# rahulaggarwal965/vslam

Hardware: AMD Instinct MI355X
Metric: frame-pairs/sec (extract+match+RANSAC) @1280×720, 2k kp, 4096 hyp; 1/2/4/8 GPU (higher is better)
Workload: dtype u8/f32/f64; 1 GPU; C3: 1280x720, 2000 keypoints, 4096 hypotheses, batch 256 pairs per GPU, SURVEY 8(d) data: rotation + parallax, sub-pixel resampling, 40-45 % outlier matches; pairs_per_gpu=256, batches_in_flight=4

## Files before the change

vslam_amd/build.py:

```python
import os
import subprocess
import sys

HERE = os.path.dirname(os.path.abspath(__file__))
CSRC = os.path.join(HERE, "csrc")
LIB = os.path.join(HERE, "libvslam_amd.so")
SOURCES = ["capi.hip", "match.hip", "ransac_sets.hip", "ransac_solve.hip", "ransac_count.hip", "ransac_select.hip", "refit.hip", "refine.hip",
           "kdtree.hip", "gray.hip", "response.hip", "select.hip", "blur.hip",
           "brief.hip", "orb_grid.hip", "pose.hip", "assoc.hip", "map.hip", "world.hip", "render.hip", "multi.hip", "pipeline.hip"]
HEADERS = ["ctx.h", "introselect.h", "image_common.h", "ransac_svd.h", "ransac_residual.h", "refine_math.h", "world_select.h",
           os.path.join("..", "..", "include", "vslam_amd.h"),
           os.path.join("..", "..", "include", "vslam_brief_pattern_31.h")]
FLAGS = ["--offload-arch=gfx950", "-O3", "-std=c++17", "-ffp-contract=off", "-fPIC", "-Wall"]
EXTRA_FLAGS = {"response.hip": ["-fno-slp-vectorize"]}
OBJDIR = os.path.join(HERE, "_obj")


EXP_LIB = os.path.join(HERE, "libvslam_amd_exp.so")
EXP_OBJDIR = os.path.join(HERE, "_obj_exp")


def _compile(hipcc, src, verbose, objdir=None, extra=()):
    objdir = objdir or OBJDIR
    obj = os.path.join(objdir, src.replace(".hip", ".o"))
    deps = [os.path.join(CSRC, src)] + [os.path.join(CSRC, h) for h in HEADERS] + [os.path.abspath(__file__)]
    if os.path.exists(obj) and all(os.path.getmtime(d) <= os.path.getmtime(obj) for d in deps):
        return obj, None
    cmd = [hipcc] + FLAGS + list(extra) + EXTRA_FLAGS.get(src, []) + ["-c", "-o", obj, src]
    if verbose:
        print(" ".join(cmd))
    return obj, subprocess.Popen(cmd, cwd=CSRC)


def build(force=False, verbose=False, experiments=False):
    hipcc = os.environ.get("HIPCC", "/opt/rocm/bin/hipcc")
    objdir, lib, extra = (EXP_OBJDIR, EXP_LIB, ("-DVSLAM_EXPERIMENTS",)) if experiments else (OBJDIR, LIB, ())
    return _build(hipcc, objdir, lib, extra, force, verbose)


def _build(hipcc, OBJDIR, LIB, extra, force, verbose):
    os.makedirs(OBJDIR, exist_ok=True)
    if force:
        for f in os.listdir(OBJDIR):
            os.remove(os.path.join(OBJDIR, f))
    jobs = [_compile(hipcc, src, verbose, OBJDIR, extra) for src in SOURCES]
    failed = [obj for obj, proc in jobs if proc is not None and proc.wait() != 0]
    if failed:
        raise subprocess.CalledProcessError(1, "hipcc -c (" + ", ".join(os.path.basename(f) for f in failed) + ")")
    objs = [obj for obj, _ in jobs]
    if os.path.exists(LIB) and all(proc is None for _, proc in jobs) and all(
            os.path.getmtime(o) <= os.path.getmtime(LIB) for o in objs):
        return LIB
    cmd = [hipcc, "--offload-arch=gfx950", "-shared", "-fPIC", "-o", LIB] + objs
    if verbose:
        print(" ".join(cmd))
    subprocess.run(cmd, check=True)
    return LIB


HOST_LIB = os.path.join(HERE, "libvslam_host.so")
HOST_SRCS = [os.path.join(HERE, "host", f) for f in ("adapters.cpp", "kdtree_nodes.cpp", "ingest.cpp", "pointmap.cpp", "display.cpp")]
HOST_HDRS = [os.path.join(HERE, "host", "host_internal.h")]
INCLUDE = os.path.join(HERE, "..", "include")


def build_host(force=False, verbose=False):
    build(force=False)
    deps = HOST_SRCS + HOST_HDRS + [LIB] + [os.path.join(INCLUDE, "vslam", f) for f in os.listdir(os.path.join(INCLUDE, "vslam"))]
    if not force and os.path.exists(HOST_LIB) and all(os.path.getmtime(d) <= os.path.getmtime(HOST_LIB) for d in deps):
        return HOST_LIB
    cmd = ["g++", "-std=c++17", "-O2", "-fPIC", "-shared", "-Wall", "-pthread", "-o", HOST_LIB] + HOST_SRCS + [
        "-L" + HERE, "-lvslam_amd", "-Wl,-rpath,$ORIGIN"]
    if verbose:
        print(" ".join(cmd))
    subprocess.run(cmd, check=True)
    return HOST_LIB


if __name__ == "__main__":
    build(force="--force" in sys.argv, verbose=True)
    build_host(force="--force" in sys.argv, verbose=True)
    build(force="--force" in sys.argv, verbose=True, experiments=True)
    print(LIB)
    print(EXP_LIB)
    print(HOST_LIB)
```

vslam_amd/capi.py:

```python
import ctypes as C
import os

_HERE = os.path.dirname(os.path.abspath(__file__))
LIB_PATH = os.environ.get("VSLAM_AMD_LIB") or os.path.join(_HERE, "libvslam_amd.so")
EXP_LIB_PATH = os.path.join(_HERE, "libvslam_amd_exp.so")

OK = 0
ERRORS = {-1: "VSLAM_ERR_INVALID", -2: "VSLAM_ERR_HIP", -3: "VSLAM_ERR_NO_DEVICE",
          -4: "VSLAM_ERR_CAPACITY", -5: "VSLAM_ERR_DEGENERATE", -6: "VSLAM_ERR_COMM"}

SYMBOLS = [
    "vslam_ctx_create", "vslam_ctx_make_current", "vslam_ctx_destroy", "vslam_ctx_set_stream", "vslam_ctx_set_option", "vslam_ctx_synchronize", "vslam_ctx_wait",
    "vslam_last_error", "vslam_ctx_workspace_bytes", "vslam_version", "vslam_brief_pattern_31", "vslam_dev_alloc", "vslam_dev_free", "vslam_copy_h2d",
    "vslam_copy_d2h", "vslam_debug_stream_copy", "vslam_debug_valu_calib", "vslam_prof_enable", "vslam_prof_reset", "vslam_prof_count", "vslam_prof_get",
    "vslam_match_knn2_ratio", "vslam_ransac_sets", "vslam_ransac_fundamental", "vslam_ransac_solve",
    "vslam_ransac_evaluate", "vslam_refit_fundamental", "vslam_refine_pairs", "vslam_kdtree_build",
    "vslam_kdtree_radius", "vslam_kdtree_nearest", "vslam_kdtree_cell_table", "vslam_extract_features", "vslam_extract_features_grid", "vslam_triangulate_points", "vslam_frontend_pairs_pose", "vslam_pipeline_batches_redone", "vslam_corner_stats", "vslam_bgr2gray", "vslam_min_eigen",
    "vslam_good_features", "vslam_gaussian7", "vslam_orb_describe", "vslam_extract_Rt", "vslam_triangulate", "vslam_associate_map_points", "vslam_reprojection_filter",
    "vslam_match_features",
    "vslam_map_create", "vslam_map_destroy", "vslam_map_reset", "vslam_map_step", "vslam_map_view", "vslam_map_observations",
    "vslam_track_sequences",
    "vslam_world_create", "vslam_world_destroy", "vslam_world_reset", "vslam_world_step", "vslam_world_lift", "vslam_world_view",
    "vslam_map_attach_world", "vslam_world_render",
    "vslam_view_default", "vslam_view_look_at", "vslam_render_points", "vslam_map_render",
# ... 49 lines not shown
    def default(cls, width, height, lib=None):
        lib = lib or load_library()
        v = cls()
        rc = lib.vslam_view_default(C.c_int(width), C.c_int(height), C.byref(v))
        if rc != OK:
            raise VslamError(f"{ERRORS.get(rc, rc)}: vslam_view_default({width}, {height})")
        return v

    @classmethod
    def look_at(cls, eye, target, up, width, height, lib=None, **fields):
        lib = lib or load_library()
        v = cls.default(width, height, lib)
        d3 = C.c_double * 3
        rc = lib.vslam_view_look_at(d3(*[float(x) for x in eye]), d3(*[float(x) for x in target]), d3(*[float(x) for x in up]), v.mv)
        if rc != OK:
            raise VslamError(f"{ERRORS.get(rc, rc)}: vslam_view_look_at({eye}, {target}, {up})")
        for k, val in fields.items():
            if k in ("background_bgr", "frustum_bgr"):
                val = (C.c_uint8 * 3)(*val)
            setattr(v, k, val)
        return v

    def copy(self, **fields):
        v = type(self).from_buffer_copy(self)
        for k, val in fields.items():
            if k in ("background_bgr", "frustum_bgr"):
                val = (C.c_uint8 * 3)(*val)
            setattr(v, k, val)
        return v


def load_library(path=LIB_PATH):
    if not os.path.exists(path):
        raise VslamError(
            f"{path} is missing: run `python -m vslam_amd.build` (hipcc, gfx950). "
            "There is no CPU fallback.")
    lib = C.CDLL(path)
    lib.vslam_last_error.restype = C.c_char_p
    lib.vslam_version.restype = C.c_char_p
    return lib


def _ptr(t):
    if t is None:
        return C.c_void_p(0)
    if isinstance(t, int):
        return C.c_void_p(t)
    return C.c_void_p(t.data_ptr())


class Context:

    def __init__(self, device=0, use_torch_stream=True, lib=None):
        import torch
        self.torch = torch
        self.lib = lib if lib is not None else load_library()
        self.handle = C.c_void_p()
        rc = self.lib.vslam_ctx_create(C.c_int(device), C.byref(self.handle))
        if rc != OK:
            raise VslamError(f"vslam_ctx_create failed: {ERRORS.get(rc, rc)} (no HIP device? there is no CPU fallback)")
        self.device = torch.device("cuda", device)
        self.own_stream = not use_torch_stream
        if use_torch_stream:
            s = torch.cuda.current_stream(self.device)
            self._check(self.lib.vslam_ctx_set_stream(self.handle, C.c_void_p(s.cuda_stream)))

    def _ready(self):
        if getattr(self, "own_stream", True):
            self.torch.cuda.current_stream(self.device).synchronize()

    def close(self):
        if self.handle:
            self.lib.vslam_ctx_destroy(self.handle)
            self.handle = C.c_void_p()

    def __del__(self):
        try:
            self.close()
        except Exception:
            pass

    def _check(self, rc):
        if rc != OK:
            msg = self.lib.vslam_last_error(self.handle)
            raise VslamError(f"{ERRORS.get(rc, rc)}: {msg.decode() if msg else ''}")

    def _dev(self, t, dtype, name):
        torch = self.torch
        if t is None:
            return None
        if not (t.is_cuda and t.dtype == dtype and t.is_contiguous()):
            raise VslamError(f"{name}: need a contiguous cuda tensor of {dtype}, got {t.dtype} on {t.device}")
        return t

    def synchronize(self):
        self._check(self.lib.vslam_ctx_synchronize(self.handle))

    def corner_stats(self):
        a = (C.c_uint64 * 5)()
        self._check(self.lib.vslam_corner_stats(self.handle, a))
        return {"frames": int(a[0]), "px_per_frame": int(a[1]), "listed_pixels": int(a[2]), "frames_overflowed": int(a[3]),
                "pool_sets": int(a[4])}

    def workspace_bytes(self):
        n = C.c_size_t()
        self._check(self.lib.vslam_ctx_workspace_bytes(self.handle, C.byref(n)))
        return n.value

    OPT_RANSAC_ALL_SUMS = 1
    OPT_RANSAC_MIN_MATCHES = 2
    OPT_RANSAC_SOLVER = 3
    OPT_MATCH_SHAPE = 4
    OPT_CORNER_WINDOW_PCT = 5
    OPT_RANSAC_MIN_ITEMS = 6
    OPT_CORNER_LIST_CAP = 7
    OPT_MATCH_FORM = 8
    OPT_TREE_FORK = 9
    OPT_POSE_REFIT = 10
    OPT_POSE_REFINE = 11

    def set_option(self, option, value):
        self._check(self.lib.vslam_ctx_set_option(self.handle, C.c_int(option), C.c_int(int(value))))

    def prof_enable(self, on=True):
        self._check(self.lib.vslam_prof_enable(self.handle, C.c_int(1 if on else 0)))

    def prof_reset(self):
        self._check(self.lib.vslam_prof_reset(self.handle))

    def prof_report(self):
        n = self.lib.vslam_prof_count(self.handle)
        if n < 0:
            self._check(n)
        out = {}
        for i in range(n):
            name = C.create_string_buffer(128)
            ms = C.c_double()
            cnt = C.c_int64()
            self._check(self.lib.vslam_prof_get(self.handle, C.c_int(i), name, C.c_int(128), C.byref(ms), C.byref(cnt)))
            out[name.value.decode()] = (ms.value, cnt.value)
        return out

    def debug_detect(self, bgr, max_corners, width=None):
        torch = self.torch
        F, H = bgr.shape[0], bgr.shape[1]
        W = width if width is not None else bgr.shape[2]
        stride = bgr.shape[2] * (bgr.shape[3] if bgr.dim() == 4 else 1)
        xy = torch.zeros((F, max_corners, 2), dtype=torch.float32, device=bgr.device)
        n = torch.zeros((F,), dtype=torch.int32, device=bgr.device)
        self._ready()
        self._check(self.lib.vslam_debug_detect(self.handle, _ptr(bgr), C.c_int(F), C.c_int(W), C.c_int(H), C.c_int(stride),
                                                C.c_int(max_corners), C.c_int(max_corners), _ptr(xy), _ptr(n)))
        return xy, n

    def debug_valu_calib(self):
        self._check(self.lib.vslam_debug_valu_calib(self.handle))

    def debug_stream_copy(self, src, dst, bytes_per_lane):
        self._check(self.lib.vslam_debug_stream_copy(self.handle, _ptr(src), _ptr(dst), C.c_size_t(src.numel() * src.element_size()),
                                                     C.c_int(bytes_per_lane)))

    def match_knn2_ratio(self, desc1, n1, desc2, n2, want_knn=False):
        torch = self.torch
        B, K, _ = desc1.shape
        self._dev(desc1, torch.uint8, "desc1"); self._dev(desc2, torch.uint8, "desc2")
        self._dev(n1, torch.int32, "n1"); self._dev(n2, torch.int32, "n2")
        pairs = torch.empty((B, K, 2), dtype=torch.int32, device=desc1.device)
        m = torch.empty((B,), dtype=torch.int32, device=desc1.device)
        knn = torch.empty((B, K, 4), dtype=torch.int32, device=desc1.device) if want_knn else None
        self._check(self.lib.vslam_match_knn2_ratio(self.handle, _ptr(desc1), _ptr(n1), _ptr(desc2), _ptr(n2),
                                                    C.c_int(B), C.c_int(K), _ptr(pairs), _ptr(m), _ptr(knn)))
        return (pairs, m, knn) if want_knn else (pairs, m)

    def ransac_sets(self, seeds, m, hyp):
        torch = self.torch
        B = seeds.shape[0]
        self._dev(seeds, torch.int32, "seeds"); self._dev(m, torch.int32, "m")
        sets = torch.empty((B, hyp, 8), dtype=torch.int32, device=seeds.device)
        draws = torch.empty((B, hyp * 8), dtype=torch.int32, device=seeds.device)
        self._check(self.lib.vslam_ransac_sets(self.handle, _ptr(seeds), _ptr(m), C.c_int(B), C.c_int(hyp),
                                               _ptr(sets), _ptr(draws)))
        return sets

    def ransac_fundamental(self, xy1, xy2, pairs, m, sets, threshold):
        torch = self.torch
        B, K, _ = xy1.shape
        H = sets.shape[1]
        dev = xy1.device
        for t, dt, nm in ((xy1, torch.float32, "xy1"), (xy2, torch.float32, "xy2"), (pairs, torch.int32, "pairs"),
                          (m, torch.int32, "m"), (sets, torch.int32, "sets")):
            self._dev(t, dt, nm)
        out = dict(
            F=torch.zeros((B, 9), dtype=torch.float32, device=dev),
            mask=torch.zeros((B, K), dtype=torch.uint8, device=dev),
            best=torch.zeros((B, 4), dtype=torch.int32, device=dev),
            matches=torch.zeros((B, K, 2), dtype=torch.int32, device=dev),
            hypF=torch.zeros((B, H, 9), dtype=torch.float32, device=dev),
            hyp_count=torch.zeros((B, H), dtype=torch.int32, device=dev),
            hyp_sum=torch.zeros((B, H), dtype=torch.float32, device=dev),
        )
        self._check(self.lib.vslam_ransac_fundamental(
            self.handle, _ptr(xy1), _ptr(xy2), _ptr(pairs), _ptr(m), _ptr(sets), C.c_int(B), C.c_int(K),
            C.c_int(H), C.c_float(threshold), _ptr(out["F"]), _ptr(out["mask"]), _ptr(out["best"]),
            _ptr(out["matches"]), _ptr(out["hypF"]), _ptr(out["hyp_count"]), _ptr(out["hyp_sum"])))
        return out

    def ransac_evaluate(self, xy1, xy2, pairs, m, hypF, threshold):
        torch = self.torch
        B, K, _ = xy1.shape
        H = hypF.shape[1]
        dev = xy1.device
        for t, dt, nm in ((xy1, torch.float32, "xy1"), (xy2, torch.float32, "xy2"), (pairs, torch.int32, "pairs"),
                          (m, torch.int32, "m"), (hypF, torch.float32, "hypF")):
            self._dev(t, dt, nm)
        out = dict(
            F=torch.zeros((B, 9), dtype=torch.float32, device=dev),
            mask=torch.zeros((B, K), dtype=torch.uint8, device=dev),
            best=torch.zeros((B, 4), dtype=torch.int32, device=dev),
            matches=torch.zeros((B, K, 2), dtype=torch.int32, device=dev),
            hyp_count=torch.zeros((B, H), dtype=torch.int32, device=dev),
            hyp_sum=torch.zeros((B, H), dtype=torch.float32, device=dev),
        )
        self._check(self.lib.vslam_ransac_evaluate(
            self.handle, _ptr(xy1), _ptr(xy2), _ptr(pairs), _ptr(m), _ptr(hypF), C.c_int(B), C.c_int(K), C.c_int(H),
            C.c_float(threshold), _ptr(out["F"]), _ptr(out["mask"]), _ptr(out["best"]), _ptr(out["matches"]),
            _ptr(out["hyp_count"]), _ptr(out["hyp_sum"])))
        return out

    def refit_fundamental(self, xy1, xy2, matches, best, F, out=None, want_stats=True):
        torch = self.torch
        B, K, _ = xy1.shape
        for t, dt, nm in ((xy1, torch.float32, "xy1"), (xy2, torch.float32, "xy2"), (matches, torch.int32, "matches"),
                          (best, torch.int32, "best"), (F, torch.float32, "F"), (out, torch.float32, "out")):
            self._dev(t, dt, nm)
        if out is None:
            out = torch.empty((B, 9), dtype=torch.float32, device=xy1.device)
        stats = torch.empty((B, 4), dtype=torch.float64, device=xy1.device) if want_stats else None
        self._ready()
        self._check(self.lib.vslam_refit_fundamental(self.handle, _ptr(xy1), _ptr(xy2), _ptr(matches), _ptr(best), C.c_int(B),
                                                     C.c_int(K), _ptr(F), _ptr(out), _ptr(stats)))
        return out, stats

    def refine_pairs(self, xy1, xy2, matches, best, K, R, t, points4d, gate_sq=16.0, max_iterations=20, want_stats=True):
        import numpy as np
        torch = self.torch
        B, Kp, _ = xy1.shape
        for x, dt, nm in ((xy1, torch.float32, "xy1"), (xy2, torch.float32, "xy2"), (matches, torch.int32, "matches"),
                          (best, torch.int32, "best"), (R, torch.float32, "R"), (t, torch.float32, "t"),
                          (points4d, torch.float32, "points4d")):
            self._dev(x, dt, nm)
        Kh = np.ascontiguousarray(np.asarray(K, np.float32).reshape(9))
        c2 = torch.empty((B, 12), dtype=torch.float32, device=xy1.device)
        stats = torch.empty((B, 4), dtype=torch.float64, device=xy1.device) if want_stats else None
        self._ready()
        self._check(self.lib.vslam_refine_pairs(self.handle, _ptr(xy1), _ptr(xy2), _ptr(matches), _ptr(best), C.c_int(B), C.c_int(Kp),
                                                Kh.ctypes.data_as(C.c_void_p), C.c_float(gate_sq), C.c_int(max_iterations),
                                                _ptr(R), _ptr(t), _ptr(c2), _ptr(points4d), _ptr(stats)))
        return R, t, c2, points4d, stats

    def kdtree_build(self, xy, n):
        torch = self.torch
        B, K, _ = xy.shape
        self._dev(xy, torch.float32, "xy"); self._dev(n, torch.int32, "n")
        nodes = torch.full((B, K), -1, dtype=torch.int32, device=xy.device)
        self._check(self.lib.vslam_kdtree_build(self.handle, _ptr(xy), _ptr(n), C.c_int(B), C.c_int(K), _ptr(nodes)))
        return nodes

    def kdtree_radius(self, nodes, xy, n, queries, nq, radius, hit_cap=8):
        torch = self.torch
        B, K, _ = xy.shape
        Q = queries.shape[1]
        self._dev(nodes, torch.int32, "nodes"); self._dev(xy, torch.float32, "xy"); self._dev(n, torch.int32, "n")
        self._dev(queries, torch.float32, "queries"); self._dev(nq, torch.int32, "nq")
        hits = torch.full((B, Q, hit_cap), -1, dtype=torch.int32, device=xy.device)
        counts = torch.zeros((B, Q), dtype=torch.int32, device=xy.device)
        self._check(self.lib.vslam_kdtree_radius(self.handle, _ptr(nodes), _ptr(xy), _ptr(n), C.c_int(B), C.c_int(K),
                                                 _ptr(queries), _ptr(nq), C.c_int(Q), C.c_float(radius),
                                                 _ptr(hits), _ptr(counts), C.c_int(hit_cap)))
        return hits, counts

    def kdtree_nearest(self, nodes, xy, n, queries, nq, max_distance_sq=float("inf")):
        torch = self.torch
        B, K, _ = xy.shape
        Q = queries.shape[1]
        best = torch.full((B, Q), -2, dtype=torch.int32, device=xy.device)
        self._check(self.lib.vslam_kdtree_nearest(self.handle, _ptr(nodes), _ptr(xy), _ptr(n), C.c_int(B), C.c_int(K),
                                                  _ptr(queries), _ptr(nq), C.c_int(Q), C.c_float(max_distance_sq),
                                                  _ptr(best)))
        return best

    def bgr2gray(self, bgr):
        torch = self.torch
        F, H, W, _ = bgr.shape
        self._dev(bgr, torch.uint8, "bgr")
        gray = torch.empty((F, H, W), dtype=torch.uint8, device=bgr.device)
        self._check(self.lib.vslam_bgr2gray(self.handle, _ptr(bgr), C.c_int(F), C.c_int(W), C.c_int(H), C.c_int(3 * W), _ptr(gray)))
        return gray

    def min_eigen(self, gray):
        torch = self.torch
        F, H, W = gray.shape
        self._dev(gray, torch.uint8, "gray")
        eig = torch.empty((F, H, W), dtype=torch.float32, device=gray.device)
        self._check(self.lib.vslam_min_eigen(self.handle, _ptr(gray), C.c_int(F), C.c_int(W), C.c_int(H), _ptr(eig)))
        return eig

# ... 740 lines not shown
```

vslam_amd/csrc/ransac_count.hip:

```cpp
#include "ransac_residual.h"

namespace {
using namespace vs_ransac;

constexpr int kCntHyps = 128;
constexpr int kCntWaves = 8;
constexpr int kCntQueue = 320;
constexpr int kCntLdsMatches = 4096;
constexpr int kScreenMatches = 128;
constexpr int kScreenHyps = 128;
constexpr int kRankThreads = 512;
constexpr int kPilotHyps = kRankThreads / 64;
constexpr int kCandMax = 8;
constexpr float kCntTinyDD = 0x1p-120f;
constexpr int kFcmpOGT = 2, kFcmpOLT = 4, kFcmpULT = 12;
constexpr int kCntRec = 12;
typedef __attribute__((address_space(3))) volatile uint32_t cnt_queue_t;
static_assert(VSLAM_MAX_KP <= 65536, "queue words keep the match index in 16 bits");

__host__ __device__ constexpr int cnt_pad(int n) { return (n + 255) & ~255; }
constexpr int kHeadUncertified = -1;
__device__ __forceinline__ float cnt_sum_rel(int adds) { return fmaxf(0x1p-18f, (float)(13 + adds) * 0x1p-24f); }

struct CntBand {
// ... 662 lines not shown
            int knext = 0;
            if (lane == 0) knext = atomicAdd(&s_next, 1);
            int hh;
            {
                int kk = k, w = 0;
                while (w + 1 < kListWaves && kk >= s_nlist[w]) kk -= s_nlist[w++];
                hh = s_list[w * 64 + kk];
            }
            bound = max(bound, *(__attribute__((address_space(3))) const volatile int *)&s_bound);
            CntRec R;
            cnt_load_record(R, s_rec, hh);
            const int word = ZERO ? 0 : s_state[hh] >> 2;
            const int head_cnt = ZERO ? 0 : *(__attribute__((address_space(3))) const volatile int *)&s_cnt[hh];
            float head_sum = ZERO ? 0.f : s_part[hh];
            int cnt = 0, pot = word & 0xFFFF, seen = org;
            bool dropped = false, unk = false;
            v2f acc;
            acc.x = 0.f;
            acc.y = 0.f;
            for (int s = 0;; s++) {
                if (s >= nsub && (ZERO || s > nsub || !(word & kHeadMine))) break;
                const bool hd = !ZERO && s == nsub;
                const int pot_walk = pot;
                const int ix = (hd ? 0 : org + s * 256) + 4 * lane;
                const int il = min(ix, mpad - 4);
                const float4 X1 = *reinterpret_cast<const float4 *>(cx1 + il), Y1 = *reinterpret_cast<const float4 *>(cy1 + il);
                const float4 X2 = *reinterpret_cast<const float4 *>(cx2 + il), Y2 = *reinterpret_cast<const float4 *>(cy2 + il);
                if (hd || (s == nsub - 1 && part)) {
                    cnt_sub_block<true>(R, X1, Y1, X2, Y2, ix, hh, lane, hd ? n0 : m, cnt, q, qn, acc, s_unk, pot, unk);
                    seen += hd ? 0 : (m - org) & 255;
                } else {
                    cnt_sub_block<false>(R, X1, Y1, X2, Y2, ix, hh, lane, m, cnt, q, qn, acc, s_unk, pot, unk);
                    seen += 256;
                }
                while (qn >= 64) {
                    cnt_drain(q, qn - 64, 64, lane, s_rec, s_cnt, cx1, cy1, cx2, cy2, threshold);
                    qn -= 64;
                }
                if (hd) {
                    head_sum = 0.f;
                    pot = pot_walk;
                    break;
                }
                if (pot + (m - seen) < bound) {
                    dropped = true;
                    break;
                }
                if (seen < m && bound == floor_count && pot + (m - seen) == bound && !unk && R.beta >= 0.f && !(word & kHeadNoSum)) {
                    const float S = head_sum + __int_as_float(__builtin_amdgcn_readlane(__float_as_int(wave_sum_to_lane63(acc.x + acc.y)), 63));
                    const float ns = (float)seen;
                    const float err = (2.02f * R.beta * sqrtf(ns * S) + ns * R.beta * R.beta + sum_rel * S) * 1.0001f;
                    const float upper = ((S + err) + threshold * (float)(m - seen)) * 1.0001f;
                    if (upper < floor_sum * 0.9999f) {
                        dropped = true;
                        break;
                    }
                }
            }
            if (dropped) {
#ifdef VSLAM_EXPERIMENTS
                if (lane == 0) s_state[hh] = 2 | (seen << 2);
#else
                if (lane == 0) s_state[hh] = 2;
#endif
            } else {
                const float part_sum = head_sum + wave_sum_to_lane63(acc.x + acc.y);
                bool beaten = false;
                if (bound == floor_count && pot == bound && !unk && R.beta >= 0.f) {
                    const float S = __int_as_float(__builtin_amdgcn_readlane(__float_as_int(part_sum), 63));
                    const float ns = (float)m;
                    const float err = (2.02f * R.beta * sqrtf(ns * S) + ns * R.beta * R.beta + sum_rel * S) * 1.0001f;
                    beaten = (S + err) * 1.0001f < floor_sum * 0.9999f;
                }
                if (lane == 63) s_part[hh] = part_sum;
                const int certain = head_cnt + cnt;
                if (beaten) {
#ifdef VSLAM_EXPERIMENTS
                    if (lane == 0) s_state[hh] = 2 | (seen << 2);
#else
                    if (lane == 0) s_state[hh] = 2;
#endif
                } else if (lane == 0) {
                    if (cnt) atomicAdd(&s_cnt[hh], cnt);
                    if (certain > bound) {
                        atomicMax(&s_bound, certain);
                        atomicMax(&cbound[b], certain);
                    }
                }
                if (!beaten) bound = max(bound, certain);
            }
            k = __builtin_amdgcn_readfirstlane(knext);
        }
        if (qn > 0) cnt_drain(q, 0, qn, lane, s_rec, s_cnt, cx1, cy1, cx2, cy2, threshold);
    }
    __syncthreads();
    if (tid < nh) {
        const int st = s_state[tid] & 3;
        hyp_count[out] = st == 1 ? s_cnt[tid] : -1;
        int nan_bits = 0x7FC00000;
#ifdef VSLAM_EXPERIMENTS
        if (exit_payload && st != 1) nan_bits |= st == 2 ? min(s_state[tid] >> 2, 0x3FFFFF) : 0x3FFFFF;
#endif
        hyp_sum[out] = __int_as_float(nan_bits);
        const float S = st == 1 ? s_part[tid] : 0.f;
        float err = INFINITY;
        if (st == 1 && my_ok && !s_unk[tid]) {
            const double Sd = (double)S;
            const double rel = (double)cnt_sum_rel(2 * ((m - (ZERO ? 0 : n0) + 255) >> 8) + 9);
            err = (float)((2.02 * my_beta * sqrt((double)m * Sd) + (double)m * my_beta * my_beta + rel * Sd) * (1.0 + 0x1p-20));
        }
        reinterpret_cast<float2 *>(approx)[out] = make_float2(S, err);
    }
}

}

int vs_launch_ransac_count(vslam_ctx *ctx, const float *xy1, const float *xy2, const int32_t *pairs, const int32_t *m,
                           const float *hypF, int batch, int kp_stride, int hyp, float threshold, int32_t *hyp_count,
                           float *hyp_sum, float *approx) {
    const int min_m = ctx->ransac_min_matches;
    int rc;
    int32_t *cbound = nullptr, *pot0 = nullptr;
    float *rk = nullptr, *cmax = nullptr;
    const int kp_pad = cnt_pad(kp_stride);
    if ((rc = vs_arena_get(ctx, "ransac.cbound", sizeof(int32_t) * (size_t)batch, (void **)&cbound))) return rc;
    unsigned long long *sfloor = nullptr;
    if ((rc = vs_arena_get(ctx, "ransac.sfloor", sizeof(unsigned long long) * (size_t)batch, (void **)&sfloor))) return rc;
    static const bool no_sum_rule = VS_EXPERIMENT_ENV("VSLAM_RANSAC_NO_SUM_RULE") != nullptr;
    const bool from_zero = VS_EXPERIMENT_ENV("VSLAM_RANSAC_COUNT_FROM_ZERO") != nullptr;
#ifdef VSLAM_EXPERIMENTS
    const int exit_payload = VS_EXPERIMENT_ENV("VSLAM_RANSAC_COUNT_EXIT_PAYLOAD") != nullptr ? 1 : 0;
#endif
    int2 *head = nullptr;
    if ((rc = vs_arena_get(ctx, "ransac.head", sizeof(int2) * (size_t)batch * hyp, (void **)&head))) return rc;
    const unsigned long long *use_floor = no_sum_rule ? nullptr : sfloor;
    if ((rc = vs_arena_get(ctx, "ransac.pot0", sizeof(int32_t) * (size_t)batch * hyp, (void **)&pot0))) return rc;
    if ((rc = vs_arena_get(ctx, "ransac.rk", sizeof(float) * 4 * (size_t)kp_pad * batch, (void **)&rk))) return rc;
    if ((rc = vs_arena_get(ctx, "ransac.cmax", sizeof(float) * 2 * (size_t)batch, (void **)&cmax))) return rc;
    {
        VsProfScope ps(ctx, "ransac_rank_kernel");
        ransac_rank_kernel<<<batch, kRankThreads, 0, ctx->stream>>>(xy1, xy2, pairs, m, min_m, kp_stride, kp_pad, hyp, threshold, hypF,
                                                                    cbound, rk, cmax, sfloor);
    }
    {
        VsProfScope ps(ctx, "ransac_screen_kernel");
        dim3 grid(vs_div_up(hyp, kScreenHyps), batch);
        ransac_screen_kernel<<<grid, 256, 0, ctx->stream>>>(rk, kp_pad, m, min_m, kp_stride, hyp, threshold, hypF, cmax, cbound, pot0, head);
    }
    {
        VsProfScope ps(ctx, "ransac_cand_kernel");
        ransac_cand_kernel<<<batch, 64 * kCandMax, 0, ctx->stream>>>(rk, kp_pad, m, min_m, kp_stride, hyp, threshold, hypF, pot0,
                                                                     no_sum_rule ? 0 : 1, cbound, sfloor);
    }
    if (int arc = vs_aux_job_point(ctx, 4)) return arc;
    {
        VsProfScope ps(ctx, "ransac_count_kernel");
        const bool lds = kp_pad <= kCntLdsMatches;
        const size_t dyn = (lds ? sizeof(float) * 4 * (size_t)kp_pad : 0) + sizeof(uint32_t) * kCntQueue * kCntWaves;
        const size_t dyn_max = sizeof(float) * 4 * kCntLdsMatches + sizeof(uint32_t) * kCntQueue * kCntWaves;
        dim3 grid(vs_div_up(hyp, kCntHyps), batch);
#ifdef VSLAM_EXPERIMENTS
        if (from_zero) {
            if (dyn > 32 * 1024 && (rc = vs_allow_dynamic_lds(ctx, ransac_count_kernel<true, true>, "ransac_count_from_zero", dyn_max)))
                return rc;
            if (lds)
                ransac_count_kernel<true, true><<<grid, 64 * kCntWaves, dyn, ctx->stream>>>(
                    rk, kp_pad, m, min_m, kp_stride, hyp, threshold, hypF, pot0, head, cmax, hyp_count, hyp_sum, approx, cbound,
                    use_floor VS_CNT_PAYLOAD_ARG);
            else
                ransac_count_kernel<false, true><<<grid, 64 * kCntWaves, dyn, ctx->stream>>>(
                    rk, kp_pad, m, min_m, kp_stride, hyp, threshold, hypF, pot0, head, cmax, hyp_count, hyp_sum, approx, cbound,
                    use_floor VS_CNT_PAYLOAD_ARG);
            return VSLAM_OK;
        }
#endif
        (void)from_zero;
        if (dyn > 32 * 1024 &&
            (rc = vs_allow_dynamic_lds(ctx, ransac_count_kernel<true, false>, "ransac_count", dyn_max)))
            return rc;
        if (lds)
            ransac_count_kernel<true, false><<<grid, 64 * kCntWaves, dyn, ctx->stream>>>(
                rk, kp_pad, m, min_m, kp_stride, hyp, threshold, hypF, pot0, head, cmax, hyp_count, hyp_sum, approx, cbound,
                    use_floor VS_CNT_PAYLOAD_ARG);
        else
            ransac_count_kernel<false, false><<<grid, 64 * kCntWaves, dyn, ctx->stream>>>(
                rk, kp_pad, m, min_m, kp_stride, hyp, threshold, hypF, pot0, head, cmax, hyp_count, hyp_sum, approx, cbound,
                    use_floor VS_CNT_PAYLOAD_ARG);
    }
    return VSLAM_OK;
}
```

vslam_amd/csrc/ransac_residual.h:

```cpp
#pragma once

#include "ctx.h"

namespace vs_ransac {

struct ResidualF {
    float f[9];
    double ft[6];
};
__device__ __forceinline__ void residual_prepare(ResidualF &R) {
    R.ft[0] = (double)R.f[0];
    R.ft[1] = (double)R.f[3];
    R.ft[2] = (double)R.f[6];
    R.ft[3] = (double)R.f[1];
    R.ft[4] = (double)R.f[4];
    R.ft[5] = (double)R.f[7];
}
__device__ __forceinline__ float residual_e(const ResidualF &R, const float4 c, const double dx2, const double dy2) {
    const float x1 = c.x, y1 = c.y, x2 = c.z, y2 = c.w;
    const float a0 = R.f[0] * x1 + R.f[1] * y1 + R.f[2];
    const float a1 = R.f[3] * x1 + R.f[4] * y1 + R.f[5];
    const float a2 = R.f[6] * x1 + R.f[7] * y1 + R.f[8];
    const float t0 = (float)(__builtin_fma(R.ft[1], dy2, R.ft[0] * dx2) + R.ft[2]);
    const float t1 = (float)(__builtin_fma(R.ft[4], dy2, R.ft[3] * dx2) + R.ft[5]);
    const float n = (x2 * a0 + y2 * a1) + a2;
    const float q = (n * n) / (a0 * a0);
    return ((q + a1 * a1) + t0 * t0) + t1 * t1;
}

typedef float v2f __attribute__((ext_vector_type(2)));
__device__ __forceinline__ v2f residual_e2(const ResidualF &R, const v2f x1, const v2f y1, const v2f x2, const v2f y2,
                                           const double2 da, const double2 db) {
    const v2f a0 = (R.f[0] * x1 + R.f[1] * y1) + R.f[2];
    const v2f a1 = (R.f[3] * x1 + R.f[4] * y1) + R.f[5];
    const v2f a2 = (R.f[6] * x1 + R.f[7] * y1) + R.f[8];
    v2f t0, t1;
    t0.x = (float)(__builtin_fma(R.ft[1], da.y, R.ft[0] * da.x) + R.ft[2]);
    t0.y = (float)(__builtin_fma(R.ft[1], db.y, R.ft[0] * db.x) + R.ft[2]);
    t1.x = (float)(__builtin_fma(R.ft[4], da.y, R.ft[3] * da.x) + R.ft[5]);
    t1.y = (float)(__builtin_fma(R.ft[4], db.y, R.ft[3] * db.x) + R.ft[5]);
    const v2f n = (x2 * a0 + y2 * a1) + a2;
    const v2f nn = n * n, dd = a0 * a0;
    v2f q;
    q.x = nn.x / dd.x;
    q.y = nn.y / dd.y;
    return ((q + a1 * a1) + t0 * t0) + t1 * t1;
}

}

int vs_launch_ransac_count(vslam_ctx *ctx, const float *xy1, const float *xy2, const int32_t *pairs, const int32_t *m,
                           const float *hypF, int batch, int kp_stride, int hyp, float threshold, int32_t *hyp_count,
                           float *hyp_sum, float *approx);
```

Measured before the change: 97420 frame-pairs/s.

## Add MFMA-based RANSAC hypothesis pruning pass before count kernel

Adds a new kernel that runs before the RANSAC count kernel. It uses 32x32x2 f32 MFMA tiles to compute epipolar numerators and denominators for 32 hypotheses against 32 matches at a time. A conservative rounding-error margin certifies definite outlier misses. Hypotheses whose certified miss count exceeds what they could afford have pot0 marked dead, so the count kernel can skip them. This trades an extra launch and a partial scan of the matches for less work in the expensive exact count, and it relies on the margin staying sound so results do not change.

```diff
diff --git a/vslam_amd/build.py b/vslam_amd/build.py
--- a/vslam_amd/build.py
+++ b/vslam_amd/build.py
@@ -5,10 +5,10 @@
 HERE = os.path.dirname(os.path.abspath(__file__))
 CSRC = os.path.join(HERE, "csrc")
 LIB = os.path.join(HERE, "libvslam_amd.so")
-SOURCES = ["capi.hip", "match.hip", "ransac_sets.hip", "ransac_solve.hip", "ransac_count.hip", "ransac_select.hip", "refit.hip", "refine.hip",
+SOURCES = ["capi.hip", "match.hip", "ransac_sets.hip", "ransac_solve.hip", "ransac_count.hip", "ransac_prune.hip", "ransac_select.hip", "refit.hip", "refine.hip",
            "kdtree.hip", "gray.hip", "response.hip", "select.hip", "blur.hip",
            "brief.hip", "orb_grid.hip", "pose.hip", "assoc.hip", "map.hip", "world.hip", "render.hip", "multi.hip", "pipeline.hip"]
-HEADERS = ["ctx.h", "introselect.h", "image_common.h", "ransac_svd.h", "ransac_residual.h", "refine_math.h", "world_select.h",
+HEADERS = ["ctx.h", "introselect.h", "image_common.h", "ransac_svd.h", "ransac_residual.h", "ransac_prune_cert.h", "refine_math.h", "world_select.h",
            os.path.join("..", "..", "include", "vslam_amd.h"),
            os.path.join("..", "..", "include", "vslam_brief_pattern_31.h")]
 FLAGS = ["--offload-arch=gfx950", "-O3", "-std=c++17", "-ffp-contract=off", "-fPIC", "-Wall"]
diff --git a/vslam_amd/capi.py b/vslam_amd/capi.py
--- a/vslam_amd/capi.py
+++ b/vslam_amd/capi.py
@@ -225,6 +225,23 @@
         self._check(self.lib.vslam_debug_detect(self.handle, _ptr(bgr), C.c_int(F), C.c_int(W), C.c_int(H), C.c_int(stride),
                                                 C.c_int(max_corners), C.c_int(max_corners), _ptr(xy), _ptr(n)))
         return xy, n
+
+    def debug_ransac_prune_x(self, batch, hyp):
+        torch = self.torch
+        x = torch.zeros((batch, hyp), dtype=torch.int32, device="cuda")
+        self._ready()
+        self._check(self.lib.vslam_debug_ransac_prune_x(self.handle, _ptr(x), C.c_int(batch), C.c_int(hyp)))
+        return x
+
+    def debug_ransac_prune_tile(self, F, xy):
+        torch = self.torch
+        self._dev(F, torch.float32, "F"); self._dev(xy, torch.float32, "xy")
+        assert tuple(F.shape) == (32, 9) and tuple(xy.shape) == (4, 32)
+        n = torch.zeros((32, 32), dtype=torch.float32, device=F.device)
+        a0 = torch.zeros((32, 32), dtype=torch.float32, device=F.device)
+        self._ready()
+        self._check(self.lib.vslam_debug_ransac_prune_tile(self.handle, _ptr(F), _ptr(xy), _ptr(n), _ptr(a0)))
+        return n, a0
 
     def debug_valu_calib(self):
         self._check(self.lib.vslam_debug_valu_calib(self.handle))
diff --git a/vslam_amd/csrc/ransac_count.hip b/vslam_amd/csrc/ransac_count.hip
--- a/vslam_amd/csrc/ransac_count.hip
+++ b/vslam_amd/csrc/ransac_count.hip
@@ -838,6 +838,8 @@
         ransac_cand_kernel<<<batch, 64 * kCandMax, 0, ctx->stream>>>(rk, kp_pad, m, min_m, kp_stride, hyp, threshold, hypF, pot0,
                                                                      no_sum_rule ? 0 : 1, cbound, sfloor);
     }
+    if ((rc = vs_launch_ransac_prune(ctx, rk, kp_pad, m, min_m, kp_stride, hyp, threshold, hypF, cmax, cbound, pot0, batch, kScreenMatches)))
+        return rc;
     if (int arc = vs_aux_job_point(ctx, 4)) return arc;
     {
         VsProfScope ps(ctx, "ransac_count_kernel");
diff --git a/vslam_amd/csrc/ransac_prune.hip b/vslam_amd/csrc/ransac_prune.hip
--- /dev/null
+++ b/vslam_amd/csrc/ransac_prune.hip
@@ -0,0 +1,193 @@
+#include "ransac_prune_cert.h"
+#include "ransac_residual.h"
+
+namespace {
+
+typedef float v16f __attribute__((ext_vector_type(16)));
+constexpr int kPruneWaves = 4;
+constexpr int kPruneHyps = 32;
+constexpr int kPruneTile = 32;
+constexpr int kPruneStep = 2;
+constexpr int kPruneOGT = 2;
+
+__host__ __device__ constexpr int prune_row(int r, int half) { return (r & 3) + 8 * (r >> 2) + 4 * half; }
+
+struct PruneA {
+    float n[5], d[2];
+};
+__device__ __forceinline__ PruneA prune_operands(const float *f, bool half) {
+    PruneA A;
+#pragma unroll
+    for (int s = 0; s < 4; s++) A.n[s] = half ? f[2 * s + 1] : f[2 * s];
+    A.n[4] = half ? 0.f : f[8];
+    A.d[0] = half ? f[1] : f[0];
+    A.d[1] = half ? 0.f : f[2];
+    return A;
+}
+
+__device__ __forceinline__ void prune_tile(const PruneA &A, bool half, float x1, float y1, float x2, float y2, v16f &n, v16f &a0) {
+    const float p = x2 * (half ? y1 : x1);
+    const float q = y2 * (half ? x1 : y1);
+    const float b1 = half ? q : x2, b2 = half ? y2 : q, b3 = half ? y1 : x1, b4 = half ? 0.f : 1.f;
+    v16f z;
+#pragma unroll
+    for (int r = 0; r < 16; r++) z[r] = 0.f;
+    n = __builtin_amdgcn_mfma_f32_32x32x2f32(A.n[0], p, z, 0, 0, 0);
+    n = __builtin_amdgcn_mfma_f32_32x32x2f32(A.n[1], b1, n, 0, 0, 0);
+    n = __builtin_amdgcn_mfma_f32_32x32x2f32(A.n[2], b2, n, 0, 0, 0);
+    n = __builtin_amdgcn_mfma_f32_32x32x2f32(A.n[3], b3, n, 0, 0, 0);
+    n = __builtin_amdgcn_mfma_f32_32x32x2f32(A.n[4], b4, n, 0, 0, 0);
+    a0 = __builtin_amdgcn_mfma_f32_32x32x2f32(A.d[0], b3, z, 0, 0, 0);
+    a0 = __builtin_amdgcn_mfma_f32_32x32x2f32(A.d[1], b4, a0, 0, 0, 0);
+}
+
+#ifdef VSLAM_EXPERIMENTS
+#define VS_PRUNE_X_PARAM , int32_t *__restrict__ x_out
+#else
+#define VS_PRUNE_X_PARAM
+#endif
+
+__global__ __launch_bounds__(64 * kPruneWaves) void ransac_prune_mfma_kernel(
+    const float *__restrict__ rk, int kp_pad, const int32_t *__restrict__ m_arr, int min_m, int kp_stride, int hyp, float threshold,
+    float splus, const float *__restrict__ hypF, const float *__restrict__ cmax, const int32_t *__restrict__ cbound, int32_t *__restrict__ pot0,
+    int n_head, int gate VS_PRUNE_X_PARAM) {
+    const int b = blockIdx.y, lane = threadIdx.x & 63, col = lane & 31;
+    const bool half = lane >= 32;
+    const int wave = __builtin_amdgcn_readfirstlane(threadIdx.x >> 6);
+    const int m = min(m_arr[b], kp_stride);
+    const int bound = cbound[b];
+    if (m < min_m) return;
+    const int n0 = min(m, n_head);
+    const int hbase = (blockIdx.x * kPruneWaves + wave) * kPruneHyps;
+    if (m <= n0 || hbase >= hyp) return;
+    if (gate && m - bound + 1 <= n0) return;
+
+    const int h = hbase + col;
+    const size_t hi = (size_t)b * hyp + min(h, hyp - 1);
+    const int behind = m - n0;
+    const int lim = pot0[hi] + behind - bound;
+    bool live0 = h < hyp && lim >= 0 && lim < behind;
+    if (__ballot(live0) == 0ull) return;
+    float f[9];
+#pragma unroll
+    for (int k = 0; k < 9; k++) f[k] = hypF[hi * 9 + k];
+    const float c = pc_margin(f, cmax[2 * b], cmax[2 * b + 1], threshold, splus);
+    live0 = live0 && c < INFINITY;
+    if (__ballot(live0) == 0ull) return;
+    const PruneA A = prune_operands(f, half);
+    float cr[16];
+#pragma unroll
+    for (int r = 0; r < 16; r++) cr[r] = __shfl(c, half ? prune_row(r, 1) : prune_row(r, 0), 64);
+
+    const float *r1 = rk + (size_t)b * 4 * kp_pad, *r2 = r1 + kp_pad, *r3 = r2 + kp_pad, *r4 = r3 + kp_pad;
+    int X[kPruneHyps], L[kPruneHyps];
+#pragma unroll
+    for (int i = 0; i < kPruneHyps; i++) {
+        X[i] = 0;
+        L[i] = __builtin_amdgcn_readlane(live0 ? lim : -1, i);
+    }
+    const int end = m;
+    for (int base = n0; base < end; base += kPruneStep * kPruneTile) {
+        float x1[kPruneStep], y1[kPruneStep], x2[kPruneStep], y2[kPruneStep];
+#pragma unroll
+        for (int t = 0; t < kPruneStep; t++) {
+            const int j = min(base + t * kPruneTile + col, m - 1);
+            x1[t] = r1[j];
+            y1[t] = r2[j];
+            x2[t] = r3[j];
+            y2[t] = r4[j];
+        }
+#pragma unroll
+        for (int t = 0; t < kPruneStep; t++) {
+            v16f n, a0;
+            prune_tile(A, half, x1[t], y1[t], x2[t], y2[t], n, a0);
+            const unsigned long long valid = __ballot(base + t * kPruneTile + col < end);
+#pragma unroll
+            for (int r = 0; r < 16; r++) {
+                const unsigned long long miss =
+                    __builtin_amdgcn_fcmpf(fabsf(n[r]), fmaf(splus, fabsf(a0[r]), cr[r]), kPruneOGT) & valid;
+                X[prune_row(r, 0)] += __popc((uint32_t)miss);
+                X[prune_row(r, 1)] += __popc((uint32_t)(miss >> 32));
+            }
+        }
+        int top = -1;
+#pragma unroll
+        for (int i = 0; i < kPruneHyps; i++) top = max(top, X[i] <= L[i] ? X[i] : -1);
+        const int seen = min(base + kPruneStep * kPruneTile, end) - n0;
+        if (top < 0 || 2 * top < seen) break;
+    }
+    int xv = 0;
+#pragma unroll
+    for (int i = 0; i < kPruneHyps; i++) xv = col == i ? X[i] : xv;
+    if (!half && h < hyp) {
+        if (live0 && xv > lim) pot0[hi] = -behind - 1;
+#ifdef VSLAM_EXPERIMENTS
+        if (x_out) x_out[hi] = xv;
+#endif
+    }
+}
+
+#ifdef VSLAM_EXPERIMENTS
+__global__ __launch_bounds__(64) void ransac_prune_tile_kernel(const float *__restrict__ F, const float *__restrict__ xy,
+                                                               float *__restrict__ n_out, float *__restrict__ a0_out) {
+    const int lane = threadIdx.x, col = lane & 31;
+    const bool half = lane >= 32;
+    float f[9];
+#pragma unroll
+    for (int k = 0; k < 9; k++) f[k] = F[col * 9 + k];
+    const PruneA A = prune_operands(f, half);
+    v16f n, a0;
+    prune_tile(A, half, xy[col], xy[32 + col], xy[64 + col], xy[96 + col], n, a0);
+#pragma unroll
+    for (int r = 0; r < 16; r++) {
+        const int row = half ? prune_row(r, 1) : prune_row(r, 0);
+        n_out[row * 32 + col] = n[r];
+        a0_out[row * 32 + col] = a0[r];
+    }
+}
+#endif
+
+}
+
+int vs_launch_ransac_prune(vslam_ctx *ctx, const float *rk, int kp_pad, const int32_t *m, int min_m, int kp_stride, int hyp,
+                           float threshold, const float *hypF, const float *cmax, const int32_t *cbound, int32_t *pot0, int batch,
+                           int n_head) {
+    if (VS_EXPERIMENT_ENV("VSLAM_RANSAC_NO_PRUNE") != nullptr) return VSLAM_OK;
+    int gate = 1;
+    if (const char *e = VS_EXPERIMENT_ENV("VSLAM_RANSAC_PRUNE_GATE")) gate = atoi(e);
+#ifdef VSLAM_EXPERIMENTS
+    int32_t *x_out = nullptr;
+    if (int rc = vs_arena_get(ctx, "ransac.prune_x", sizeof(int32_t) * (size_t)batch * hyp, (void **)&x_out)) return rc;
+    VS_HIP(ctx, hipMemsetAsync(x_out, 0, sizeof(int32_t) * (size_t)batch * hyp, ctx->stream));
+#endif
+    VsProfScope ps(ctx, "ransac_prune_kernel");
+    dim3 grid(vs_div_up(hyp, kPruneWaves * kPruneHyps), batch);
+#ifdef VSLAM_EXPERIMENTS
+    ransac_prune_mfma_kernel<<<grid, 64 * kPruneWaves, 0, ctx->stream>>>(rk, kp_pad, m, min_m, kp_stride, hyp, threshold, pc_splus(threshold), hypF, cmax,
+                                                                         cbound, pot0, n_head, gate, x_out);
+#else
+    ransac_prune_mfma_kernel<<<grid, 64 * kPruneWaves, 0, ctx->stream>>>(rk, kp_pad, m, min_m, kp_stride, hyp, threshold, pc_splus(threshold), hypF, cmax,
+                                                                         cbound, pot0, n_head, gate);
+#endif
+    return VSLAM_OK;
+}
+
+#ifdef VSLAM_EXPERIMENTS
+extern "C" {
+int vslam_debug_ransac_prune_x(vslam_ctx *ctx, int32_t *d_out, int batch, int hyp) {
+    if (!ctx) return VSLAM_ERR_INVALID;
+    VS_REQUIRE(ctx, d_out && batch > 0 && hyp > 0 && vs_ptr_bits(d_out) % 4 == 0, VSLAM_ERR_INVALID);
+    const size_t bytes = sizeof(int32_t) * (size_t)batch * hyp;
+    const auto it = ctx->arena.find("ransac.prune_x");
+    VS_REQUIRE(ctx, it != ctx->arena.end() && it->second.bytes >= bytes, VSLAM_ERR_INVALID);
+    VS_HIP(ctx, hipMemcpyAsync(d_out, it->second.ptr, bytes, hipMemcpyDeviceToDevice, ctx->stream));
+    return VSLAM_OK;
+}
+int vslam_debug_ransac_prune_tile(vslam_ctx *ctx, const float *d_F, const float *d_xy, float *d_n, float *d_a0) {
+    if (!ctx) return VSLAM_ERR_INVALID;
+    VS_REQUIRE(ctx, d_F && d_xy && d_n && d_a0 && vs_ptr_bits(d_F, d_xy, d_n, d_a0) % 4 == 0, VSLAM_ERR_INVALID);
+    ransac_prune_tile_kernel<<<1, 64, 0, ctx->stream>>>(d_F, d_xy, d_n, d_a0);
+    return VSLAM_OK;
+}
+}
+#endif
diff --git a/vslam_amd/csrc/ransac_prune_cert.h b/vslam_amd/csrc/ransac_prune_cert.h
--- /dev/null
+++ b/vslam_amd/csrc/ransac_prune_cert.h
@@ -0,0 +1,40 @@
+#pragma once
+
+#include <cmath>
+
+#if defined(__HIPCC__)
+#define PC_HD __host__ __device__ inline
+#else
+#define PC_HD inline
+#endif
+
+#if defined(__clang__)
+#pragma clang fp contract(off)
+#endif
+
+constexpr double kPcNumer = 18.0, kPcDenom = 7.0;
+constexpr double kPcU = 0x1p-24, kPcFloor = 0x1p-40;
+
+PC_HD float pc_splus(float thr) { return (float)(sqrt((double)thr) * (1.0 + 0x1p-20)); }
+
+PC_HD bool pc_pair_ok(float C1, float C2, float thr) {
+    return thr >= 0x1p-20f && thr <= 0x1p20f && C1 <= 0x1p20f && C2 <= 0x1p20f && C1 >= 0.f && C2 >= 0.f;
+}
+
+PC_HD float pc_margin(const float *f, float C1, float C2, float thr, float splus) {
+    float big = 0.f;
+    bool finite = true;
+    for (int k = 0; k < 9; k++) {
+        big = fmaxf(big, fabsf(f[k]));
+        finite = finite && f[k] == f[k];
+    }
+    if (!(pc_pair_ok(C1, C2, thr) && finite && big <= 1024.f)) return INFINITY;
+    const float c21 = C2 * C1;
+    const float T = (((fabsf(f[0]) + fabsf(f[1])) + (fabsf(f[3]) + fabsf(f[4]))) * c21 + (fabsf(f[2]) + fabsf(f[5])) * C2) +
+                    ((fabsf(f[6]) + fabsf(f[7])) * C1 + fabsf(f[8]));
+    const float T0 = (fabsf(f[0]) + fabsf(f[1])) * C1 + fabsf(f[2]);
+    const float E = (float)(kPcNumer * kPcU) * T, E0 = (float)(kPcDenom * kPcU) * T0;
+    return (E + splus * E0) * (1.f + 0x1p-18f) + (float)kPcFloor;
+}
+
+PC_HD bool pc_miss(float n, float a0, float splus, float c) { return fabsf(n) > fmaf(splus, fabsf(a0), c); }
diff --git a/vslam_amd/csrc/ransac_residual.h b/vslam_amd/csrc/ransac_residual.h
--- a/vslam_amd/csrc/ransac_residual.h
+++ b/vslam_amd/csrc/ransac_residual.h
@@ -52,3 +52,7 @@
 int vs_launch_ransac_count(vslam_ctx *ctx, const float *xy1, const float *xy2, const int32_t *pairs, const int32_t *m,
                            const float *hypF, int batch, int kp_stride, int hyp, float threshold, int32_t *hyp_count,
                            float *hyp_sum, float *approx);
+
+int vs_launch_ransac_prune(vslam_ctx *ctx, const float *rk, int kp_pad, const int32_t *m, int min_m, int kp_stride, int hyp,
+                           float threshold, const float *hypF, const float *cmax, const int32_t *cbound, int32_t *pot0, int batch,
+                           int n_head);
```

Result: faster. 102,600 frame-pairs/s, median of 6 (+5.3%).
